# antoniorizzoeng/climate-sim-mpi-cpp

Hardware: AMD Instinct MI355X
Metric: Mcell-updates/sec (16384^2 fp64 advection-diffusion sweep) (higher is better)
Workload: dtype f64

## Files before the change

### climate-sim-mpi-cpp_amd/csrc/api.cpp

```cpp
#include "stepper.hpp"

namespace csim {

static thread_local std::string g_err;
int fail(int code, const std::string& msg) {
    g_err = msg;
    return code;
}
static bool pow2(double x) {
    if (!(x > 0.0) || !std::isnormal(x)) return false;
    int e = 0;
    return std::frexp(x, &e) == 0.5 && std::isnormal(1.0 / x);
}

Phys make_phys(double dx, double dy, double D, double dt, double vx, double vy, bool contract) {
    Phys p;
    p.kdiff = dt * D;
    p.mdt = -dt;
    p.vx = vx;
    p.vy = vy;
    p.dx = dx;
    p.dy = dy;
    p.dx2 = dx * dx;
    p.dy2 = dy * dy;
    p.rdx = 1.0 / dx;
    p.rdy = 1.0 / dy;
    p.rdx2 = 1.0 / p.dx2;
    p.rdy2 = 1.0 / p.dy2;
    if (dx == 1.0 && dy == 1.0)
        p.div_mode = 0;
    else if (pow2(dx) && pow2(dy) && pow2(p.dx2) && pow2(p.dy2))
        p.div_mode = 1;
    else
        p.div_mode = 2;
    {
        const long double kx = static_cast<long double>(dt) * D / (static_cast<long double>(dx) * dx);
        const long double ky = static_cast<long double>(dt) * D / (static_cast<long double>(dy) * dy);
        const long double cx = static_cast<long double>(dt) * vx / dx, cy = static_cast<long double>(dt) * vy / dy;
        const long double acx = cx < 0 ? -cx : cx, acy = cy < 0 ? -cy : cy;
        p.a0 = static_cast<double>(1.0L - 2.0L * kx - 2.0L * ky - acx - acy);
        p.aW = static_cast<double>(kx + (vx >= 0.0 ? acx : 0.0L));
        p.aE = static_cast<double>(kx + (vx >= 0.0 ? 0.0L : acx));
        p.aS = static_cast<double>(ky + (vy >= 0.0 ? acy : 0.0L));
        p.aN = static_cast<double>(ky + (vy >= 0.0 ? 0.0L : acy));
    }
    {
        const double g = (1.0 + 4.0 * std::fabs(p.kdiff) * (1.0 / p.dx2 + 1.0 / p.dy2) +
                          2.0 * std::fabs(p.mdt) * (std::fabs(vx) / std::fabs(dx) + std::fabs(vy) / std::fabs(dy))) * (1.0 + 1e-9);
        const double thr = std::ldexp(1.0, 1022) / std::pow(g, MAX_FUSE);
        p.fast_thr = (std::isfinite(g) && thr >= std::ldexp(1.0, 900)) ? thr : 0.0;
    }
    p.slow_thr = p.p2_hi = p.p2_q = p.p2_k = 0.0;
    if (!contract && p.div_mode <= 1 && p.fast_thr > 0.0 && pow2(std::fabs(vx)) && pow2(std::fabs(vy)) && std::isfinite(p.kdiff) &&
        std::isfinite(p.mdt)) {
        const double A = p.div_mode == 1 ? vx * p.rdx : vx, B = p.div_mode == 1 ? vy * p.rdy : vy;
        if (pow2(std::fabs(A)) && pow2(std::fabs(B))) {
            const bool by_y = vy > 0.0 || vx < 0.0;
            const double q = by_y ? A / B : B / A, K = p.mdt * (by_y ? B : A);
            const int eA = std::ilogb(A), eB = std::ilogb(B), eq = std::ilogb(q);
            int e2 = 0, ew = std::min({0, eA, eB, eq, -eq}), eh = std::max({0, eA, eB, eq, -eq});
            if (p.div_mode == 1) {
                e2 = std::min({0, std::ilogb(p.rdx2), std::ilogb(p.rdy2)});
                ew = std::min({ew, e2, std::ilogb(p.rdx), std::ilogb(p.rdy)});
                eh = std::max({eh, std::ilogb(p.rdx), std::ilogb(p.rdy)});
            }
            int er = 0;
            if (p.kdiff != 0.0) er = std::min(er, std::ilogb(p.kdiff) - 52 + e2);
            if (p.mdt != 0.0) er = std::min(er, std::ilogb(p.mdt) - 52 + std::min(eA, eB));
            const int eL = -1074 + 52 - MAX_FUSE * er - ew;
            if (eL <= -300 && eh <= 100 && pow2(std::fabs(q)) && (K == 0.0 || std::isnormal(K))) {
                p.slow_thr = std::ldexp(1.0, eL);
                p.p2_hi = std::ldexp(p.fast_thr, -(eh + 2));
                p.p2_q = q;
                p.p2_k = K;
            }
        }
    }
    if (contract) p.div_mode = 3;
    return p;
}

int fold_partials(const double* scratch_dev, int rows, int kind, double* out, hipStream_t st, const Members& mb) {
    const size_t G = static_cast<size_t>(reduce_blocks(rows, mb.cap)), hi = G * mb.count;
    std::vector<double> h(kind == 0 ? 2 * hi : hi);
    CSIM_HIP(hipMemcpyAsync(h.data(), scratch_dev, sizeof(double) * h.size(), hipMemcpyDeviceToHost, st));
    CSIM_HIP(hipStreamSynchronize(st));
    for (int m = 0; m < mb.count; ++m) {
        const double* p = h.data() + m * G;
        double r0 = p[0], r1 = kind == 0 ? p[hi] : 0.0;
        for (size_t k = 1; k < G; ++k) {
            if (kind == 0) {
                r0 = std::fmin(r0, p[k]);
                r1 = std::fmax(r1, p[hi + k]);
            } else if (kind == 1) {
                r0 += p[k];
            } else {
                r0 = max_nan(r0, p[k]);
            }
        }
        if (kind == 0) {
            out[2 * m] = r0;
            out[2 * m + 1] = r1;
        } else {
            out[m] = r0;
        }
    }
    return CSIM_OK;
}

int fold_checksum(const double* scratch_dev, int rows, unsigned long long* out, hipStream_t st, const Members& mb) {
    const size_t G = static_cast<size_t>(reduce_blocks(rows, mb.cap));
    std::vector<unsigned long long> h(G * mb.count);
    CSIM_HIP(hipMemcpyAsync(h.data(), scratch_dev, sizeof(unsigned long long) * h.size(), hipMemcpyDeviceToHost, st));
    CSIM_HIP(hipStreamSynchronize(st));
    for (int m = 0; m < mb.count; ++m) {
        unsigned long long acc = 0;
        for (size_t k = 0; k < G; ++k) acc += h[m * G + k];
        out[m] = acc;
    }
    return CSIM_OK;
}

int upload_2d(double* d, int nx, int ny, int pitch, const double* host) {
    CSIM_HIP(hipMemcpy2D(d + (LPAD - 1), sizeof(double) * pitch, host, sizeof(double) * (nx + 2),
                         sizeof(double) * (nx + 2), ny + 2, hipMemcpyHostToDevice));
    return CSIM_OK;
}
int download_2d(const double* d, int nx, int ny, int pitch, double* host) {
    CSIM_HIP(hipMemcpy2D(host, sizeof(double) * (nx + 2), d + (LPAD - 1), sizeof(double) * pitch,
                         sizeof(double) * (nx + 2), ny + 2, hipMemcpyDeviceToHost));
    return CSIM_OK;
}
int download_interior_2d(const double* d, int nx, int ny, int pitch, double* host) {
    CSIM_HIP(hipMemcpy2D(host, sizeof(double) * nx, d + pitch + LPAD, sizeof(double) * pitch,
                         sizeof(double) * nx, ny, hipMemcpyDeviceToHost));
    return CSIM_OK;
}

void neighbours8(const csim_decomp& dec, int nbr8[8]) {
    for (int k = 0; k < 4; ++k) nbr8[k] = dec.nbr[k];
    const int cx = dec.coords[0], cy = dec.coords[1], py = dec.dims[1];
    auto diag = [&](int sx, int sy, int dx_, int dy_) {
        if (dec.nbr[sx] < 0 || dec.nbr[sy] < 0) return -1;
        return dec.size == 1 ? 0 : (cx + dx_) * py + (cy + dy_);
    };
    nbr8[4] = diag(CSIM_LEFT, CSIM_BOTTOM, -1, -1);
    nbr8[5] = diag(CSIM_RIGHT, CSIM_BOTTOM, +1, -1);
    nbr8[6] = diag(CSIM_LEFT, CSIM_TOP, -1, +1);
    nbr8[7] = diag(CSIM_RIGHT, CSIM_TOP, +1, +1);
}

size_t face_doubles(int d, int H, int nx, int ny) {
    if (H == 1) return d < 2 ? static_cast<size_t>(ny) : static_cast<size_t>(nx);
    return d < 2 ? static_cast<size_t>(H) * (ny + 2) : d < 4 ? static_cast<size_t>(H) * (nx + 2)
                                                       : static_cast<size_t>(H) * H;
}

bool valid_bc(const int bc[4]) {
    for (int s = 0; s < 4; ++s)
        if (bc[s] < CSIM_BC_DIRICHLET || bc[s] > CSIM_BC_PERIODIC) return false;
    return true;
}

}

using namespace csim;

extern "C" {

const char* csim_last_error(void) { return g_err.c_str(); }

int csim_abi_version(void) { return CSIM_ABI_VERSION; }

int csim_device_count(int* count) {
    CSIM_REQUIRE(count, "count is null");
    CSIM_HIP(hipGetDeviceCount(count));
    return CSIM_OK;
}

int csim_set_device(int device) {
    CSIM_HIP(hipSetDevice(device));
    return CSIM_OK;
}

int csim_device_name(char* buf, size_t n) {
    CSIM_REQUIRE(buf && n > 0, "bad buffer");
    int dev = 0;
    CSIM_HIP(hipGetDevice(&dev));
    hipDeviceProp_t prop;
    CSIM_HIP(hipGetDeviceProperties(&prop, dev));
    std::snprintf(buf, n, "%s", prop.gcnArchName);
    return CSIM_OK;
}

int csim_pow2_velocity_screen(double dx, double dy, double D, double dt, double vx, double vy, double out[4]) {
    CSIM_REQUIRE(out, "null argument");
    const Phys p = make_phys(dx, dy, D, dt, vx, vy);
    out[0] = p.slow_thr, out[1] = p.p2_hi, out[2] = p.p2_q, out[3] = p.p2_k;
    return CSIM_OK;
}

double csim_safe_dt(double dx, double dy, double vx, double vy, double D) {
    const double inf = std::numeric_limits<double>::infinity();
    const double ax = std::fabs(vx), ay = std::fabs(vy);
    const double rate = (ax > 0 ? ax / dx : 0.0) + (ay > 0 ? ay / dy : 0.0);
    const double dt_adv = rate > 0 ? 1.0 / rate : inf;
    const double w = 1.0 / (dx * dx) + 1.0 / (dy * dy);
    const double dt_diff = D > 0 ? 1.0 / (2.0 * D * w) : inf;
    return std::min(dt_adv, dt_diff);
}

int csim_decomp_init(int size, int rank, int nx_global, int ny_global, csim_decomp* out) {
    CSIM_REQUIRE(out, "out is null");
    CSIM_REQUIRE(size >= 1 && rank >= 0 && rank < size, "bad size/rank");
    CSIM_REQUIRE(nx_global > 0 && ny_global > 0, "nx/ny must be > 0");
    int small = 1;
    for (int f = 1; static_cast<long>(f) * f <= size; ++f)
        if (size % f == 0) small = f;
    csim_decomp d{};
    d.size = size;
    d.rank = rank;
    d.dims[0] = size / small;
    d.dims[1] = small;
    d.coords[0] = rank / d.dims[1];
    d.coords[1] = rank % d.dims[1];
    const int cx = d.coords[0], cy = d.coords[1];
    d.nbr[CSIM_LEFT] = cx > 0 ? (cx - 1) * d.dims[1] + cy : CSIM_NO_NEIGHBOR;
    d.nbr[CSIM_RIGHT] = cx + 1 < d.dims[0] ? (cx + 1) * d.dims[1] + cy : CSIM_NO_NEIGHBOR;
    d.nbr[CSIM_BOTTOM] = cy > 0 ? cx * d.dims[1] + (cy - 1) : CSIM_NO_NEIGHBOR;
    d.nbr[CSIM_TOP] = cy + 1 < d.dims[1] ? cx * d.dims[1] + (cy + 1) : CSIM_NO_NEIGHBOR;
    d.nx_global = nx_global;
    d.ny_global = ny_global;
    const int bx = nx_global / d.dims[0], by = ny_global / d.dims[1];
    d.nx_local = bx + (cx == d.dims[0] - 1 ? nx_global % d.dims[0] : 0);
    d.ny_local = by + (cy == d.dims[1] - 1 ? ny_global % d.dims[1] : 0);
    d.x_offset = cx * bx;
    d.y_offset = cy * by;
    CSIM_REQUIRE(d.nx_local > 0 && d.ny_local > 0, "more ranks than cells along an axis");
    *out = d;
    return CSIM_OK;
}

int csim_exchange_plan(const csim_decomp* dec, int depth, csim_msg sends[8], int* nsend, csim_msg recvs[8],
                       int* nrecv) {
    CSIM_REQUIRE(dec && sends && nsend && recvs && nrecv, "null argument");
    CSIM_REQUIRE(depth >= 1 && depth <= MAX_FUSE, "depth must be 1..7");
    static const int recv_order1[4] = {CSIM_RIGHT, CSIM_LEFT, CSIM_TOP, CSIM_BOTTOM};
    static const int recv_order8[8] = {1, 0, 3, 2, 7, 6, 5, 4};
    int nbr8[8];
    neighbours8(*dec, nbr8);
    const int ndir = depth == 1 ? 4 : 8;
    const int* order = depth == 1 ? recv_order1 : recv_order8;
    int ns = 0, nr = 0;
    for (int d = 0; d < ndir; ++d)
        if (nbr8[d] >= 0)
            sends[ns++] = csim_msg{nbr8[d], d, static_cast<long>(face_doubles(d, depth, dec->nx_local, dec->ny_local))};
    for (int q = 0; q < ndir; ++q) {
        const int d = order[q];
        if (nbr8[d] >= 0)
            recvs[nr++] = csim_msg{nbr8[d], d, static_cast<long>(face_doubles(d, depth, dec->nx_local, dec->ny_local))};
    }
    *nsend = ns;
    *nrecv = nr;
    return CSIM_OK;
}

struct FieldMem : csim_field {
    DeviceBuf mem, partials;
    void release() { mem.release(), partials.release(); }
};
static FieldMem* owner(csim_field* f) { return static_cast<FieldMem*>(f); }

static int field_alloc(FieldMem* f) {
    CSIM_TRY(f->mem.reserve(f->bytes()));
    CSIM_HIP(hipMemset(f->mem.p, 0, f->bytes()));
    CSIM_TRY(f->partials.reserve(sizeof(double) * 2 * REDUCE_BLOCKS));
    f->alloc = f->mem.as();
    f->d = f->alloc + static_cast<size_t>(GHOST_EXTRA) * f->pitch;
    f->scratch = f->partials.as();
    return CSIM_OK;
}

int csim_field_create(int nx, int ny, int halo, double dx, double dy, csim_field** out) {
    CSIM_REQUIRE(out, "out is null");
    *out = nullptr;
    CSIM_REQUIRE(nx > 0 && ny > 0, "nx/ny must be > 0");
    CSIM_REQUIRE(halo == 1, "only halo == 1 is supported (reference src/main.cpp:65)");
    CSIM_REQUIRE(dx > 0 && dy > 0, "dx/dy must be > 0");
    FieldMem* f = new FieldMem;
    f->nx = nx;
    f->ny = ny;
    f->halo = halo;
    f->dx = dx;
    f->dy = dy;
    f->pitch = pitch_for(nx);
    if (field_alloc(f) != CSIM_OK) {
        const std::string why = g_err;
        csim_field_destroy(f);
        return fail(CSIM_ERR_HIP, "csim_field_create: " + why);
    }
    *out = f;
    return CSIM_OK;
}

int csim_field_destroy(csim_field* f) {
    if (!f) return CSIM_OK;
    owner(f)->release();
    delete owner(f);
    return CSIM_OK;
}

int csim_field_upload(csim_field* f, const double* host) {
    CSIM_REQUIRE(f && host, "null argument");
    return upload_2d(f->d, f->nx, f->ny, f->pitch, host);
}

int csim_field_download(const csim_field* f, double* host) {
    CSIM_REQUIRE(f && host, "null argument");
    return download_2d(f->d, f->nx, f->ny, f->pitch, host);
}

int csim_field_download_interior(const csim_field* f, double* host) {
    CSIM_REQUIRE(f && host, "null argument");
    return download_interior_2d(f->d, f->nx, f->ny, f->pitch, host);
}

int csim_field_fill(csim_field* f, double value) {
    CSIM_REQUIRE(f, "null field");
    CSIM_HIP(launch_fill(f->d, f->nx, f->ny, f->pitch, value, nullptr));
    CSIM_HIP(hipStreamSynchronize(nullptr));
    return CSIM_OK;
}

static bool same_shape(const csim_field* a, const csim_field* b) {
    return a && b && a->nx == b->nx && a->ny == b->ny;
}

int csim_field_copy(csim_field* dst, const csim_field* src) {
    CSIM_REQUIRE(same_shape(dst, src), "fields differ in shape");
    CSIM_HIP(hipMemcpy(dst->alloc, src->alloc, src->bytes(), hipMemcpyDeviceToDevice));
    return CSIM_OK;
}

int csim_field_swap(csim_field* a, csim_field* b) {
    CSIM_REQUIRE(same_shape(a, b), "fields differ in shape");
    std::swap(owner(a)->mem, owner(b)->mem);
    std::swap(a->alloc, b->alloc);
    std::swap(a->d, b->d);
    return CSIM_OK;
}

int csim_field_minmax(const csim_field* f, double out[2]) {
    CSIM_REQUIRE(f && out, "null argument");
    CSIM_HIP(launch_minmax(f->d, f->nx, f->ny, f->pitch, f->scratch, nullptr));
    return fold_partials(f->scratch, f->ny + 2, 0, out, nullptr);
}

int csim_field_sum(const csim_field* f, double* out) {
    CSIM_REQUIRE(f && out, "null argument");
    CSIM_HIP(launch_sum(f->d, f->nx, f->ny, f->pitch, f->scratch, nullptr));
    return fold_partials(f->scratch, f->ny, 1, out, nullptr);
}

int csim_field_linf_diff(const csim_field* a, const csim_field* b, double* out) {
    CSIM_REQUIRE(same_shape(a, b) && out, "fields differ in shape");
    CSIM_HIP(launch_linf(a->d, b->d, a->nx, a->ny, a->pitch, a->scratch, nullptr));
    return fold_partials(a->scratch, a->ny, 2, out, nullptr);
}

int csim_apply_boundary(csim_field* f, const int bc[4], const int is_physical[4], double value) {
    CSIM_REQUIRE(f && bc && is_physical, "null argument");
    CSIM_REQUIRE(valid_bc(bc), "unknown boundary type");
    GhostArgs g{};
    for (int s = 0; s < 4; ++s) {
        g.bc[s] = bc[s];
        g.phys[s] = is_physical[s] != 0;
        g.recv[s] = nullptr;
    }
    g.value = value;
    CSIM_HIP(launch_ghost_fill(f->d, nullptr, f->nx, f->ny, f->pitch, g, nullptr));
    CSIM_HIP(hipStreamSynchronize(nullptr));
    return CSIM_OK;
}

int csim_diffusion_step(const csim_field* u, csim_field* out, double D, double dt) {
    CSIM_REQUIRE(same_shape(u, out), "fields differ in shape");
    CSIM_REQUIRE(u->d != out->d, "u and out must be distinct fields");
    const Phys p = make_phys(u->dx, u->dy, D, dt, 0.0, 0.0);
    CSIM_HIP(launch_diffusion_only(u->d, out->d, u->nx, u->ny, u->pitch, p, nullptr));
    CSIM_HIP(launch_ring_copy(u->d, out->d, u->nx, u->ny, u->pitch, nullptr));
    CSIM_HIP(hipStreamSynchronize(nullptr));
    return CSIM_OK;
}

int csim_advection_step(const csim_field* u, csim_field* out, double vx, double vy, double dt) {
    CSIM_REQUIRE(same_shape(u, out), "fields differ in shape");
    CSIM_REQUIRE(u->d != out->d, "u and out must be distinct fields");
    const Phys p = make_phys(u->dx, u->dy, 0.0, dt, vx, vy);
    CSIM_HIP(launch_advection_only(u->d, out->d, u->nx, u->ny, u->pitch, p, nullptr));
    CSIM_HIP(hipStreamSynchronize(nullptr));
    return CSIM_OK;
}

int csim_fused_step(const csim_field* u, csim_field* out, double D, double dt, double vx, double vy) {
    CSIM_REQUIRE(same_shape(u, out), "fields differ in shape");
    CSIM_REQUIRE(u->d != out->d, "u and out must be distinct fields");
    const Phys p = make_phys(u->dx, u->dy, D, dt, vx, vy);
    SweepCfg cfg;
    CSIM_HIP(launch_ring_copy(u->d, out->d, u->nx, u->ny, u->pitch, nullptr));
    CSIM_HIP(launch_sweep(u->d, out->d, u->nx, u->ny, u->pitch, p, cfg, nullptr));
    CSIM_HIP(hipStreamSynchronize(nullptr));
    return CSIM_OK;
}

}
```

### climate-sim-mpi-cpp_amd/csrc/sweepO.hpp

```cpp
#pragma once
#include "sweep_core.hpp"

#pragma clang fp contract(off)

namespace csim {

__device__ __forceinline__ void face_store_cell(const FrameSync& fs, int i, int j, double v, int nx, int ny) {
    const int H = fs.face_depth;
    const unsigned long long bits = static_cast<unsigned long long>(__double_as_longlong(v));
    auto put = [&](double* face, int idx) {
        __hip_atomic_store(reinterpret_cast<unsigned long long*>(face + idx), bits, __ATOMIC_RELAXED, __HIP_MEMORY_SCOPE_AGENT);
    };
    const bool in_i = i >= 1 && i <= nx, in_j = j >= 1 && j <= ny;
    const bool l = in_i && i <= H, r = in_i && i >= nx - H + 1, b = in_j && j <= H, t = in_j && j >= ny - H + 1;
    const int cl = i - 1, cr = i - (nx - H + 1), rb = j - 1, rt = j - (ny - H + 1);
    if (l && fs.face[0]) put(fs.face[0], cl * (ny + 2) + j);
    if (r && fs.face[1]) put(fs.face[1], cr * (ny + 2) + j);
    if (b && fs.face[2]) put(fs.face[2], rb * (nx + 2) + i);
    if (t && fs.face[3]) put(fs.face[3], rt * (nx + 2) + i);
    if (l && b && fs.face[4]) put(fs.face[4], rb * H + cl);
    if (r && b && fs.face[5]) put(fs.face[5], rb * H + cr);
    if (l && t && fs.face[6]) put(fs.face[6], rt * H + cl);
    if (r && t && fs.face[7]) put(fs.face[7], rt * H + cr);
}

#ifdef CSIM_TRACE
__device__ unsigned long long* g_wave_trace = nullptr;
struct WaveTrace {
    int slot, lane;
    unsigned long long t0;
    __device__ WaveTrace(int s, int l) : slot(s), lane(l), t0(wall_clock64()) {}
    __device__ ~WaveTrace() {
        if (lane == 0 && g_wave_trace) {
            g_wave_trace[3 * slot] = t0;
            g_wave_trace[3 * slot + 1] = wall_clock64();
            g_wave_trace[3 * slot + 2] = (static_cast<unsigned long long>(__builtin_amdgcn_s_getreg(63508)) << 32) |
                                         static_cast<unsigned>(__builtin_amdgcn_s_getreg(63492));
        }
    }
};
#endif

template <int DIV, int T, int SX, int SY>
__global__ __launch_bounds__(256) void k_sweepO_dpp(const double* __restrict__ in, double* __restrict__ out, SweepArgs a) {
    constexpr int TP = OverlapGeom<T>::TP;
    constexpr int STRIDE = OverlapGeom<T>::STRIDE;
    const int nx = a.nx, ny = a.ny, pitch = a.pitch, nstrips = a.nstrips;
    const LateArgs late = LateArgs::get();
    const int lane = threadIdx.x & 63;
    const int wave = __builtin_amdgcn_readfirstlane(threadIdx.x >> 6);
#ifdef CSIM_TRACE
    WaveTrace trace_scope(blockIdx.x * 4 + wave, lane);
#endif
    int tile;
    bool frame_tile = false;
    {
        const int b = blockIdx.x;
        if (b < a.tl.frame_blocks) {
            tile = 4 * b + wave;
            if (tile >= a.tl.frame_tiles) return;
            frame_tile = true;
        } else {
            const int lb = b - a.tl.frame_blocks, nb_mid = gridDim.x - a.tl.frame_blocks - a.tl.tail_blocks;
            tile = a.tl.frame_tiles + (lb < nb_mid ? xcd_remap(lb, nb_mid, a.swz) : lb) * 4 + wave;
        }
    }
    if (tile >= a.tl.ntiles) return;
    int t0 = 0, strip0 = a.tl.r[0].strip0, nstrip = a.tl.r[0].nstrip, j0 = a.tl.r[0].j0, j1 = a.tl.r[0].j1, ry = a.tl.r[0].ry;
#pragma unroll
    for (int q = 1; q < 8; ++q)
        if (q < a.tl.nregions && tile >= a.tl.r[q - 1].t_end) {
            t0 = a.tl.r[q - 1].t_end;
            strip0 = a.tl.r[q].strip0, nstrip = a.tl.r[q].nstrip, j0 = a.tl.r[q].j0, j1 = a.tl.r[q].j1, ry = a.tl.r[q].ry;
        }
    const int local = tile - t0;
    const int strip = strip0 + local % nstrip;
    const int chunk = local / nstrip;
    const bool first = strip == 0, last = strip == nstrips - 1;
    const int jb = j0 + chunk * ry;
    const int je = min(jb + ry - 1, j1);
    const int g0 = strip * STRIDE - TP;
    const int kl = first ? a.bc.kind[CSIM_LEFT] : 3;
    const int kr = g0 + WAVE_COLS > nx ? a.bc.kind[CSIM_RIGHT] : 3;
    const int kb = a.bc.kind[CSIM_BOTTOM], kt = a.bc.kind[CSIM_TOP];
    const bool fin_frame = a.fin.line[CSIM_BOTTOM] != nullptr && (first || last || jb == 1 || je == ny);
    const bool edge = kl != 3 || kr != 3 || (kb != 3 && jb - (T - 1) < 1) || (kt != 3 && je + (T - 1) > ny) || fin_frame;
    if (frame_tile && a.fs.prio) __builtin_amdgcn_s_setprio(3);
    const bool signalling = frame_tile && a.fs.flag != nullptr;
    const bool wt = signalling && a.fs.fence == 0;
    if (edge) {
        __builtin_amdgcn_s_setprio(3);
        const bool rows = (kb != 3 && jb - (T - 1) < 1) || (kt != 3 && je + (T - 1) > ny);
        int col_case = 0;
        if (kl != 3 && kr != 3)
            col_case = 7;
        else if (kl != 3)
            col_case = kl == CSIM_BC_NEUMANN ? 2 : 1;
        else if (kr != 3)
            col_case = (kr == CSIM_BC_NEUMANN ? 5 : 3) + (nx & 1);
        if (!SPECIALISE_EDGES<DIV, T>::value || rows || col_case == 7) col_case = -1;
#define CSIM_MARCH(MODE_) \
    sweepO_march<DIV, T, MODE_, SX, SY>(in, out, nx, ny, pitch, jb, je, g0, lane, kl, kr, a.p, kb, kt, late, fin_frame, first, last, wt)
        switch (col_case) {
            case 0: if (SPECIALISE_EDGES<DIV, T>::value) CSIM_MARCH(0); break;
            case 1: if (SPECIALISE_EDGES<DIV, T>::value) CSIM_MARCH(1); break;
            case 2: if (SPECIALISE_EDGES<DIV, T>::value) CSIM_MARCH(2); break;
            case 3: if (SPECIALISE_EDGES<DIV, T>::value) CSIM_MARCH(3); break;
            case 4: if (SPECIALISE_EDGES<DIV, T>::value) CSIM_MARCH(4); break;
            case 5: if (SPECIALISE_EDGES<DIV, T>::value) CSIM_MARCH(5); break;
            case 6: if (SPECIALISE_EDGES<DIV, T>::value) CSIM_MARCH(6); break;
            default: CSIM_MARCH(M_GENERIC); break;
        }
    } else {
        bool redo = true;
        if (DIV != 3 && a.p.fast_thr > 0.0) {
            if constexpr (P2_BODY<DIV, T, SX, SY>::value) {
                if (a.p.slow_thr > 0.0) {
                    keep_branch();
                    redo = CSIM_MARCH(M_FAST_P2);
                } else {
                    redo = CSIM_MARCH(M_FAST);
                }
            } else {
                redo = CSIM_MARCH(M_FAST);
            }
        }
        if (redo) {
            keep_branch();
            CSIM_MARCH(M_PLAIN);
        }
    }
#undef CSIM_MARCH
    if (signalling) {
        const LateArgs::Ptr ka = late.here();
        FrameSync fs;
        fs.counter = ka->fs.counter, fs.flag = ka->fs.flag, fs.pass = ka->fs.pass, fs.nframe = ka->fs.nframe;
        fs.fence = ka->fs.fence, fs.face_depth = ka->fs.face_depth;
#pragma unroll
        for (int d = 0; d < 8; ++d) fs.face[d] = ka->fs.face[d];
        if (fs.fence == 0)
            asm volatile("s_waitcnt vmcnt(0)" ::: "memory");
        if (fs.fence == 0 && fs.face_depth > 0) {
            const int H = fs.face_depth;
            const int gx = g0 + 2 * lane;
            const bool out_lane = 2 * lane >= TP && 2 * lane < TP + STRIDE && gx < nx;
            const bool rows_near = jb <= H || je >= ny - H + 1;
            const bool cols_near = g0 + TP < H || g0 + TP + STRIDE > nx - H;
            if (rows_near || cols_near) {
                const int jf0 = jb == 1 ? 0 : jb, jf1 = je == ny ? ny + 1 : je;
                auto ldf = [&](const double* q) {
                    return __longlong_as_double(static_cast<long long>(__hip_atomic_load(
                        reinterpret_cast<const unsigned long long*>(q), __ATOMIC_RELAXED, __HIP_MEMORY_SCOPE_AGENT)));
                };
                for (int rho = jf0; rho <= jf1; ++rho) {
                    if (!out_lane) continue;
                    const double* src = out + static_cast<ptrdiff_t>(rho) * pitch + LPAD + gx;
                    face_store_cell(fs, gx + 1, rho, ldf(src), nx, ny);
                    if (gx + 1 < nx) face_store_cell(fs, gx + 2, rho, ldf(src + 1), nx, ny);
                    if (gx == 0) face_store_cell(fs, 0, rho, ldf(src - 1), nx, ny);
                    if (gx + 1 == nx) face_store_cell(fs, nx + 1, rho, ldf(src + 1), nx, ny);
                    if (gx + 2 == nx) face_store_cell(fs, nx + 1, rho, ldf(src + 2), nx, ny);
                }
                asm volatile("s_waitcnt vmcnt(0)" ::: "memory");
            }
        }
        if (fs.fence == 1) __threadfence();
        if (lane == 0) {
            const unsigned done = atomicAdd(fs.counter, 1u);
            if (done == fs.nframe - 1) {
                atomicExch(fs.counter, 0u);
                __hip_atomic_store(fs.flag, fs.pass, __ATOMIC_RELEASE, __HIP_MEMORY_SCOPE_SYSTEM);
            }
        }
    }
}


template <int DIV, int T>
hipError_t sweepO_div(const double* in, double* out, int pitch, const Phys& p, const SweepCfg& cfg, const Bc2& bc,
                      const FinLines& fin, const SweepPlan& plan, hipStream_t st, FrameSync fs) {
    if (plan.empty) return hipSuccess;
    if (plan.signals)
        fs.nframe = plan.nframe;
    else
        fs = FrameSync{};
    const dim3 grid(plan.nblocks), block(256);
    SweepArgs ka;
    ka.nx = plan.nx, ka.ny = plan.ny, ka.pitch = pitch, ka.nstrips = plan.nstrips, ka.swz = cfg.xcd_swizzle;
    ka.tl = plan.tl, ka.p = p, ka.bc = bc, ka.fin = fin, ka.fs = fs;
#define CSIM_LAUNCH_O(SXV, SYV) \
    hipLaunchKernelGGL((k_sweepO_dpp<DIV, T, SXV, SYV>), grid, block, cfg.lds_bytes, st, in, out, ka)
#ifdef CSIM_ISA_PROBE
    CSIM_LAUNCH_O(1, 1);
#else
    if (DIV == 3) {
        CSIM_LAUNCH_O(1, 1);
    } else {
        switch (sign_class(p)) {
            case 8: if constexpr (DIV <= 1) CSIM_LAUNCH_O(2, 2); break;
            case 7: if constexpr (DIV <= 1) CSIM_LAUNCH_O(2, 1); break;
            case 6: if constexpr (DIV <= 1) CSIM_LAUNCH_O(2, 0); break;
            case 5: if constexpr (DIV <= 1) CSIM_LAUNCH_O(1, 2); break;
            case 2: if constexpr (DIV <= 1) CSIM_LAUNCH_O(0, 2); break;
            case 4: CSIM_LAUNCH_O(1, 1); break;
            case 3: CSIM_LAUNCH_O(1, 0); break;
            case 1: CSIM_LAUNCH_O(0, 1); break;
            default: CSIM_LAUNCH_O(0, 0); break;
        }
    }
#endif
#undef CSIM_LAUNCH_O
    return hipGetLastError();
}

template <int T>
hipError_t sweepO_T(const double* in, double* out, int pitch, const Phys& p, const SweepCfg& cfg, const Bc2& bc,
                    const FinLines& fin, const SweepPlan& plan, hipStream_t st, const FrameSync& fs) {
#ifdef CSIM_ISA_PROBE
    if (p.div_mode != 0) return hipErrorInvalidValue;
    return sweepO_div<0, T>(in, out, pitch, p, cfg, bc, fin, plan, st, fs);
#else
    switch (p.div_mode) {
        case 0: return sweepO_div<0, T>(in, out, pitch, p, cfg, bc, fin, plan, st, fs);
        case 1: return sweepO_div<1, T>(in, out, pitch, p, cfg, bc, fin, plan, st, fs);
        case 3: return sweepO_div<3, T>(in, out, pitch, p, cfg, bc, fin, plan, st, fs);
        default: return sweepO_div<2, T>(in, out, pitch, p, cfg, bc, fin, plan, st, fs);
    }
#endif
}

}
```

### climate-sim-mpi-cpp_amd/csrc/sweep_core.hpp

```cpp
#pragma once
#include <algorithm>
#include <type_traits>

#include "internal.hpp"

#pragma clang fp contract(off)

namespace csim {

template <int DIV, bool FAST = false>
__device__ __forceinline__ double diffuse_term(double c, double W, double E, double S, double N,
                                               const Phys& p) {
    double lx, ly;
    if (FAST) {
        lx = __builtin_fma(-2.0, c, E) + W;
        ly = __builtin_fma(-2.0, c, N) + S;
    } else {
        const double tc = 2.0 * c;
        lx = (E - tc) + W;
        ly = (N - tc) + S;
    }
    if (DIV == 1) {
        lx = lx * p.rdx2;
        ly = ly * p.rdy2;
    } else if (DIV == 2) {
        lx = lx / p.dx2;
        ly = ly / p.dy2;
    }
    const double lap = lx + ly;
    return c + p.kdiff * lap;
}

template <int DIV, int SX = -1, int SY = -1>
__device__ __forceinline__ double advect_term(double c, double W, double E, double S, double N,
                                              const Phys& p) {
    double gx, gy;
    if (SX == 1)
        gx = c - W;
    else if (SX == 0)
        gx = E - c;
    else
        gx = (p.vx >= 0.0) ? (c - W) : (E - c);
    if (SY == 1)
        gy = c - S;
    else if (SY == 0)
        gy = N - c;
    else
        gy = (p.vy >= 0.0) ? (c - S) : (N - c);
    if (DIV == 1) {
        gx = gx * p.rdx;
        gy = gy * p.rdy;
    } else if (DIV == 2) {
        gx = gx / p.dx;
        gy = gy / p.dy;
    }
    const double adv = p.vx * gx + p.vy * gy;
    return p.mdt * adv;
}

template <int DIV, int SX = -1, int SY = -1, bool FAST = false, bool P2 = false>
__device__ __forceinline__ double cell(double c, double W, double E, double S, double N,
                                       const Phys& p) {
    if (DIV == 3) {
        double o = p.a0 * c;
        o = __builtin_fma(p.aW, W, o);
        o = __builtin_fma(p.aE, E, o);
        o = __builtin_fma(p.aS, S, o);
        return __builtin_fma(p.aN, N, o);
    }
    const double o = diffuse_term<DIV, FAST>(c, W, E, S, N, p);
    if (P2) {
        static_assert(!P2 || (FAST && DIV <= 1 && (SX == 0 || SX == 1) && (SY == 0 || SY == 1)), "see P2 above");
        const double gx = SX == 1 ? c - W : E - c;
        const double gy = SY == 1 ? c - S : N - c;
        const double F = (SY == 1 || SX == 0) ? __builtin_fma(p.p2_q, gx, gy) : __builtin_fma(p.p2_q, gy, gx);
        return o + p.p2_k * F;
    }
    if (FAST && (SX == 2 || SY == 2)) {
        if (SX == 2 && SY == 2) return o;
        double g;
        if (SY == 2)
            g = SX == 1 ? c - W : E - c;
        else
            g = SY == 1 ? c - S : N - c;
        if (DIV == 1) g = g * (SY == 2 ? p.rdx : p.rdy);
        const double adv = (SY == 2 ? p.vx : p.vy) * g;
        return o + p.mdt * adv;
    }
    return o + advect_term<DIV, (SX == 2 ? 1 : SX), (SY == 2 ? 1 : SY)>(c, W, E, S, N, p);
}

__device__ __forceinline__ double from_prev_lane(double src, double edge) {
    int lo = __builtin_amdgcn_update_dpp(__double2loint(edge), __double2loint(src), 0x138, 0xf, 0xf, false);
    int hi = __builtin_amdgcn_update_dpp(__double2hiint(edge), __double2hiint(src), 0x138, 0xf, 0xf, false);
    return __hiloint2double(hi, lo);
}
__device__ __forceinline__ double from_next_lane(double src, double edge) {
    int lo = __builtin_amdgcn_update_dpp(__double2loint(edge), __double2loint(src), 0x130, 0xf, 0xf, false);
    int hi = __builtin_amdgcn_update_dpp(__double2hiint(edge), __double2hiint(src), 0x130, 0xf, 0xf, false);
    return __hiloint2double(hi, lo);
}

__device__ __forceinline__ int xcd_remap(int b, int nb, int enable) {
    if (!enable || nb < 16) return b;
    const int per = nb >> 3, rem = nb & 7;
    const int xcd = b & 7, q = b >> 3;
    return xcd < rem ? xcd * (per + 1) + q : rem * (per + 1) + (xcd - rem) * per + q;
}

__device__ __forceinline__ void store_pair_wt(double* dst, double ox, double oy, int nvalid) {
    if (nvalid >= 1)
        __hip_atomic_store(reinterpret_cast<unsigned long long*>(dst), static_cast<unsigned long long>(__double_as_longlong(ox)),
                           __ATOMIC_RELAXED, __HIP_MEMORY_SCOPE_AGENT);
    if (nvalid >= 2)
        __hip_atomic_store(reinterpret_cast<unsigned long long*>(dst + 1), static_cast<unsigned long long>(__double_as_longlong(oy)),
                           __ATOMIC_RELAXED, __HIP_MEMORY_SCOPE_AGENT);
}

__device__ __forceinline__ void store_pair(double* dst, double ox, double oy, int nvalid) {
    if (nvalid >= 2) {
        *reinterpret_cast<double2*>(dst) = make_double2(ox, oy);
    } else if (nvalid == 1) {
        dst[0] = ox;
    }
}

struct Bc2 {
    int kind[4];
    double value;
};

__device__ __forceinline__ double shift_from_prev(double src) {
    int lo = __builtin_amdgcn_update_dpp(0, __double2loint(src), 0x138, 0xf, 0xf, true);
    int hi = __builtin_amdgcn_update_dpp(0, __double2hiint(src), 0x138, 0xf, 0xf, true);
    return __hiloint2double(hi, lo);
}
__device__ __forceinline__ double shift_from_next(double src) {
    int lo = __builtin_amdgcn_update_dpp(0, __double2loint(src), 0x130, 0xf, 0xf, true);
    int hi = __builtin_amdgcn_update_dpp(0, __double2hiint(src), 0x130, 0xf, 0xf, true);
    return __hiloint2double(hi, lo);
}

__device__ __forceinline__ void keep_branch() { asm volatile(""); }

struct FinLines {
    double* line[4];
};

struct SweepArgs {
    int nx, ny, pitch, nstrips, swz;
    Tiling tl;
    Phys p;
    Bc2 bc;
    FinLines fin;
    FrameSync fs;
};
constexpr int SWEEP_ARGS_KERNARG_OFFSET = 16;
static_assert(alignof(SweepArgs) <= 8 && 2 * sizeof(void*) == SWEEP_ARGS_KERNARG_OFFSET,
              "LateArgs reads SweepArgs from the kernel-argument segment right behind the two field pointers");

struct LateArgs {
    typedef const SweepArgs __attribute__((address_space(4))) * Ptr;
    Ptr a;
    __device__ __forceinline__ static LateArgs get() {
        typedef const char __attribute__((address_space(4))) * Bytes;
        LateArgs l;
        l.a = (Ptr)((Bytes)__builtin_amdgcn_kernarg_segment_ptr() + SWEEP_ARGS_KERNARG_OFFSET);
        return l;
    }
    __device__ __forceinline__ Ptr here() const {
        Ptr q = a;
        asm volatile("" : "+s"(q));
        return q;
    }
    __device__ __forceinline__ double* fin_line(int side) const { return here()->fin.line[side]; }
};

template <int T>
struct OverlapGeom {
    static constexpr int TP = strip_overlap(T);
    static constexpr int STRIDE = strip_stride(T);
};

__device__ __forceinline__ void pin(double& v) { asm volatile("" : "+v"(v)); }
__device__ __forceinline__ void pin2(double2& v) { asm volatile("" : "+v"(v.x), "+v"(v.y)); }

constexpr int M_FAST_P2 = -4, M_FAST = -3, M_PLAIN = -2, M_GENERIC = -1;

template <int DIV, int T, int MODE, int SX, int SY>
__device__ __forceinline__ bool sweepO_march(const double* __restrict__ in, double* __restrict__ out,
                                             int nx, int ny, int pitch, int jb, int je, int g0, int lane,
                                             int kl, int kr, const Phys& p, int kb, int kt,
                                             LateArgs late, bool fin_any, bool fin_l, bool fin_r, bool wt) {
    constexpr int TP = OverlapGeom<T>::TP;
    constexpr int STRIDE = OverlapGeom<T>::STRIDE;
    constexpr bool EDGE = MODE >= M_GENERIC, P2 = MODE == M_FAST_P2, FAST = MODE == M_FAST || P2, GENERIC = MODE == M_GENERIC;
    constexpr int CASE = MODE;
    const int gx = g0 + 2 * lane, gy = gx + 1;
    const ptrdiff_t xoff = LPAD + gx;
    const bool out_lane = 2 * lane >= TP && 2 * lane < TP + STRIDE && gx < nx;
    const int nvalid = nx - gx;
    const bool ghost_ly = kl != 3 && gy == -1;
    const bool ghost_rx = kr != 3 && gx == nx, ghost_ry = kr != 3 && gy == nx;
    const bool right_in_x = (nx & 1) == 0;
    const bool ghost_cols = kl != 3 || kr != 3;

    auto load = [&](int j) {
        return *reinterpret_cast<const double2*>(in + static_cast<ptrdiff_t>(j) * pitch + xoff);
    };

    const int r_first = jb - (T - 1);
    const int niter = (je - jb + 1) + 2 * (T - 1);
    const int last_row = r_first + niter;
    double2 L0[6];
    double2 L[T][3];
#pragma unroll
    for (int q = 0; q < 6; ++q) L0[q] = load(min(r_first - 1 + q, last_row));
    bool big = false;
    auto screen = [&](const double2& v) {
        big |= !(__builtin_fabs(v.x) < (P2 ? p.p2_hi : p.fast_thr));
        big |= !(__builtin_fabs(v.y) < (P2 ? p.p2_hi : p.fast_thr));
        if (P2) {
            big |= __builtin_fabs(v.x) < p.slow_thr && v.x != 0.0;
            big |= __builtin_fabs(v.y) < p.slow_thr && v.y != 0.0;
        }
        if (SX == 2 || SY == 2 || (P2 && SX == 0 && SY == 0)) {
            big |= __builtin_amdgcn_class(v.x, 0x20);
            big |= __builtin_amdgcn_class(v.y, 0x20);
        }
    };
    if (FAST) {
        screen(L0[0]);
        screen(L0[1]);
    }
#pragma unroll
    for (int l = 0; l < T; ++l)
#pragma unroll
        for (int q = 0; q < 3; ++q) L[l][q] = make_double2(0.0, 0.0);

    auto group = [&](auto gtag, int k0) {
        constexpr int G = decltype(gtag)::value;
        const bool rows_here = GENERIC && ((kb != 3 && k0 <= 2 * T - 2 - jb) || (kt != 3 && k0 + 5 >= ny + T - jb));
#pragma unroll
        for (int u = 0; u < 6; ++u) {
            {
                const int r = r_first + k0 + u;
#pragma unroll
                for (int l = 1; l <= T; ++l) {
                    if (G < 2 && 6 * G + u < 2 * (l - 1)) continue;
                    const int rho = r - l + 1;
                    const double2 s = (l == 1) ? L0[u % 6] : L[l - 1][(u + 1) % 3];
                    const double2 c = (l == 1) ? L0[(u + 1) % 6] : L[l - 1][(u + 2) % 3];
                    const double2 n = (l == 1) ? L0[(u + 2) % 6] : L[l - 1][u % 3];
                    double2 o;
                    {
                        const double Wx = shift_from_prev(c.y);
                        const double Ey = shift_from_next(c.x);
                        o.x = cell<DIV, SX, SY, FAST, P2>(c.x, Wx, c.y, s.x, n.x, p);
                        o.y = cell<DIV, SX, SY, FAST, P2>(c.y, c.x, Ey, s.y, n.y, p);
                        if (FAST && l == 1) screen(n);
                    }
                    if (EDGE && !GENERIC && l < T) {
                        if (CASE == 1) o.y = ghost_ly ? c.y : o.y;
                        if (CASE == 2) {
                            const double nb = shift_from_next(o.x);
                            o.y = ghost_ly ? nb : o.y;
                        }
                        if (CASE == 3) o.x = ghost_rx ? c.x : o.x;
                        if (CASE == 4) o.y = ghost_ry ? c.y : o.y;
                        if (CASE == 5) {
                            const double pb = shift_from_prev(o.y);
                            o.x = ghost_rx ? pb : o.x;
                        }
                        if (CASE == 6) o.y = ghost_ry ? o.x : o.y;
                    }
                    if (GENERIC && l < T) {
                        bool ghost_row = false;
                        if (rows_here) {
                            const bool gb = rho == 0 && kb != 3, gt = rho == ny + 1 && kt != 3;
                            ghost_row = gb || gt;
                            if (ghost_row) {
                                const int kk = gb ? kb : kt;
                                if (kk != CSIM_BC_NEUMANN) {
                                    double2 t = c;
                                    pin2(t);
                                    o = t;
                                } else if (gt) {
                                    double2 t = L[l][(u + 2) % 3];
                                    pin2(t);
                                    o = t;
                                }
                            }
                        }
                        if (!ghost_row && ghost_cols) {
                            if (kl == CSIM_BC_NEUMANN) {
                                double t = o.x;
                                pin(t);
                                const double nb = shift_from_next(t);
                                o.y = ghost_ly ? nb : o.y;
                            } else if (kl != 3) {
                                double t = c.y;
                                pin(t);
                                o.y = ghost_ly ? t : o.y;
                            }
                            if (kr == CSIM_BC_NEUMANN) {
                                if (right_in_x) {
                                    double t = o.y;
                                    pin(t);
                                    const double pb = shift_from_prev(t);
                                    o.x = ghost_rx ? pb : o.x;
                                } else {
                                    double t = o.x;
                                    pin(t);
                                    o.y = ghost_ry ? t : o.y;
                                }
                            } else if (kr != 3) {
                                if (right_in_x) {
                                    double t = c.x;
                                    pin(t);
                                    o.x = ghost_rx ? t : o.x;
                                } else {
                                    double t = c.y;
                                    pin(t);
                                    o.y = ghost_ry ? t : o.y;
                                }
                            }
                        }
                    }
                    if (EDGE && T >= 2 && l == T - 1 && fin_any) {
                        keep_branch();
                        if (rho >= jb && rho <= je) {
                            if (fin_l && (kl != 3 ? gx == 0 : gy == -1)) late.fin_line(CSIM_LEFT)[rho - 1] = kl != 3 ? o.x : o.y;
                            if (fin_r) {
                                const int col = kr != 3 ? nx - 1 : nx;
                                if (gx == col) late.fin_line(CSIM_RIGHT)[rho - 1] = o.x;
                                if (gy == col) late.fin_line(CSIM_RIGHT)[rho - 1] = o.y;
                            }
                        }
                        if (jb == 1 && rho == (kb != 3 ? 1 : 0) && out_lane) store_pair(late.fin_line(CSIM_BOTTOM) + gx, o.x, o.y, nvalid);
                        if (je == ny && rho == (kt != 3 ? ny : ny + 1) && out_lane) store_pair(late.fin_line(CSIM_TOP) + gx, o.x, o.y, nvalid);
                    }
                    if (l < T) {
                        if (GENERIC && rows_here && rho == 1 && kb == CSIM_BC_NEUMANN) {
                            double2 t = o;
                            pin2(t);
                            L[l][(u + 2) % 3] = t;
                        }
                        L[l][u % 3] = o;
                    } else if (rho >= jb && rho <= je && out_lane) {
                        if (wt) {
                            keep_branch();
                            store_pair_wt(out + static_cast<ptrdiff_t>(rho) * pitch + xoff, o.x, o.y, nvalid);
                        } else {
                            store_pair(out + static_cast<ptrdiff_t>(rho) * pitch + xoff, o.x, o.y, nvalid);
                        }
                    }
                }
                L0[u % 6] = load(min(r + 5, last_row));
            }
        }
    };
    using G2 = std::integral_constant<int, 2>;
    if (EDGE) {
        for (int k0 = 0; k0 < niter; k0 += 6) group(G2{}, k0);
    } else {
        group(std::integral_constant<int, 0>{}, 0);
        if (niter > 6) group(std::integral_constant<int, 1>{}, 6);
        for (int k0 = 12; k0 < niter; k0 += 6) group(G2{}, k0);
    }
    return FAST && __builtin_amdgcn_ballot_w64(big) != 0;
}

template <int DIV, int T>
struct SPECIALISE_EDGES {
    static constexpr bool value = specialise_edges(DIV, T);
};

template <int DIV, int T, int SX, int SY>
struct P2_BODY {
    static constexpr bool value = SPECIALISE_EDGES<DIV, T>::value && (SX == 0 || SX == 1) && (SY == 0 || SY == 1);
};

struct GhostDev {
    int bc[4];
    int phys[4];
    double value;
    const double* recv[4];
    const double* adj[4];
    int ext_depth;
};

__device__ __forceinline__ size_t at(int i, int j, int pitch) {
    return static_cast<size_t>(j) * pitch + (LPAD - 1) + i;
}

__device__ __forceinline__ void ghost_fill_cell(double* __restrict__ a, double* __restrict__ b, int nx, int ny,
                                                int pitch, const GhostDev& g, int t) {
    auto put = [&](size_t o, double v) {
        a[o] = v;
        if (b) b[o] = v;
    };
    if (t < ny) {
        const int j = t + 1;
        for (int s = CSIM_LEFT; s <= CSIM_RIGHT; ++s) {
            const int ig = s == CSIM_LEFT ? 0 : nx + 1;
            const int ia = s == CSIM_LEFT ? 1 : nx;
            if (g.phys[s]) {
                if (g.bc[s] == CSIM_BC_DIRICHLET)
                    put(at(ig, j, pitch), g.value);
                else if (g.bc[s] == CSIM_BC_NEUMANN)
                    put(at(ig, j, pitch), g.adj[s] ? g.adj[s][t] : a[at(ia, j, pitch)]);
            } else if (g.recv[s]) {
                put(at(ig, j, pitch), g.recv[s][t]);
            }
        }
    }
    if (t < nx) {
        const int i = t + 1;
        for (int s = CSIM_BOTTOM; s <= CSIM_TOP; ++s) {
            const int jg = s == CSIM_BOTTOM ? 0 : ny + 1;
            const int ja = s == CSIM_BOTTOM ? 1 : ny;
            if (g.phys[s]) {
                if (g.bc[s] == CSIM_BC_DIRICHLET)
                    put(at(i, jg, pitch), g.value);
                else if (g.bc[s] == CSIM_BC_NEUMANN)
                    put(at(i, jg, pitch), g.adj[s] ? g.adj[s][t] : a[at(i, ja, pitch)]);
            } else if (g.recv[s]) {
                put(at(i, jg, pitch), g.recv[s][t]);
            }
        }
    }
    const int tc = nx > ny ? nx : ny;
    if (t == tc) {
        for (int cs = CSIM_LEFT; cs <= CSIM_RIGHT; ++cs) {
            const int ig = cs == CSIM_LEFT ? 0 : nx + 1;
            const int ia = cs == CSIM_LEFT ? 1 : nx;
            for (int rs = CSIM_BOTTOM; rs <= CSIM_TOP; ++rs) {
                const int jg = rs == CSIM_BOTTOM ? 0 : ny + 1;
                const int ja = rs == CSIM_BOTTOM ? 1 : ny;
                const bool row_d = g.phys[rs] && g.bc[rs] == CSIM_BC_DIRICHLET;
                const bool row_n = g.phys[rs] && g.bc[rs] == CSIM_BC_NEUMANN;
                const bool col_d = g.phys[cs] && g.bc[cs] == CSIM_BC_DIRICHLET;
                const bool col_n = g.phys[cs] && g.bc[cs] == CSIM_BC_NEUMANN;
                if (row_d) {
                    put(at(ig, jg, pitch), g.value);
                } else if (row_n) {
                    double v;
                    if (col_d)
                        v = g.value;
                    else if (col_n)
                        v = g.adj[cs] ? g.adj[cs][ja - 1] : a[at(ia, ja, pitch)];
                    else if (!g.phys[cs] && g.recv[cs])
                        v = g.recv[cs][ja - 1];
                    else
                        v = a[at(ig, ja, pitch)];
                    put(at(ig, jg, pitch), v);
                } else if (col_d) {
                    put(at(ig, jg, pitch), g.value);
                } else if (col_n) {
                    double v;
                    if (!g.phys[rs] && g.recv[rs])
                        v = g.recv[rs][ia - 1];
                    else
                        v = a[at(ia, jg, pitch)];
                    put(at(ig, jg, pitch), v);
                }
            }
        }
    }
}

}
```

Before: 1.670 million.

## Screen P2 fast path with integer bit-range accumulators and full-wave vector stores

Result: no change. 1.662 million (-0.5%).

```diff
diff --git a/climate-sim-mpi-cpp_amd/csrc/api.cpp b/climate-sim-mpi-cpp_amd/csrc/api.cpp
--- a/climate-sim-mpi-cpp_amd/csrc/api.cpp
+++ b/climate-sim-mpi-cpp_amd/csrc/api.cpp
@@ -70,7 +70,7 @@
             const int eL = -1074 + 52 - MAX_FUSE * er - ew;
             if (eL <= -300 && eh <= 100 && pow2(std::fabs(q)) && (K == 0.0 || std::isnormal(K))) {
                 p.slow_thr = std::ldexp(1.0, eL);
-                p.p2_hi = std::ldexp(p.fast_thr, -(eh + 2));
+                p.p2_hi = std::ldexp(1.0, std::ilogb(p.fast_thr) - (eh + 2));
                 p.p2_q = q;
                 p.p2_k = K;
             }
diff --git a/climate-sim-mpi-cpp_amd/csrc/p2_screen.hpp b/climate-sim-mpi-cpp_amd/csrc/p2_screen.hpp
--- /dev/null
+++ b/climate-sim-mpi-cpp_amd/csrc/p2_screen.hpp
@@ -0,0 +1,64 @@
+#pragma once
+#include <cstdint>
+#include <cstring>
+
+#if defined(__HIPCC__) || defined(__CUDACC__)
+#define CSIM_HD __host__ __device__ __forceinline__
+#else
+#define CSIM_HD inline
+#endif
+
+namespace csim {
+
+struct P2Acc {
+    uint32_t tmin;
+    int32_t smax;
+    uint32_t umax;
+    int32_t smin;
+};
+
+CSIM_HD P2Acc p2_acc_init() { return P2Acc{0xffffffffu, 0, 0u, 0}; }
+
+CSIM_HD uint64_t p2_bits(double v) {
+#if defined(__HIP_DEVICE_COMPILE__)
+    return static_cast<uint64_t>(__double_as_longlong(v));
+#else
+    uint64_t b;
+    std::memcpy(&b, &v, sizeof b);
+    return b;
+#endif
+}
+
+CSIM_HD uint32_t p2_min3(uint32_t a, uint32_t b, uint32_t c) { return (a < b ? a : b) < c ? (a < b ? a : b) : c; }
+CSIM_HD uint32_t p2_max3(uint32_t a, uint32_t b, uint32_t c) { return (a > b ? a : b) > c ? (a > b ? a : b) : c; }
+CSIM_HD int32_t p2_min3(int32_t a, int32_t b, int32_t c) { return (a < b ? a : b) < c ? (a < b ? a : b) : c; }
+CSIM_HD int32_t p2_max3(int32_t a, int32_t b, int32_t c) { return (a > b ? a : b) > c ? (a > b ? a : b) : c; }
+
+template <bool NEG0>
+CSIM_HD void p2_acc_pair(P2Acc& a, double x, double y) {
+    const uint64_t bx = p2_bits(x), by = p2_bits(y);
+    const uint32_t hx = static_cast<uint32_t>(bx >> 32), hy = static_cast<uint32_t>(by >> 32);
+    const uint32_t tx = static_cast<uint32_t>(((bx << 1) - 1) >> 32), ty = static_cast<uint32_t>(((by << 1) - 1) >> 32);
+    a.tmin = p2_min3(a.tmin, tx, ty);
+    a.smax = p2_max3(a.smax, static_cast<int32_t>(hx), static_cast<int32_t>(hy));
+    a.umax = p2_max3(a.umax, hx, hy);
+    if (NEG0) a.smin = p2_min3(a.smin, static_cast<int32_t>(hx), static_cast<int32_t>(hy));
+}
+
+template <bool NEG0>
+CSIM_HD bool p2_rejects(const P2Acc& a, double slow_thr, double p2_hi) {
+    const uint32_t lo2 = static_cast<uint32_t>((p2_bits(slow_thr) << 1) >> 32);
+    const uint32_t hi = static_cast<uint32_t>(p2_bits(p2_hi) >> 32);
+    bool bad = a.tmin < lo2 || a.smax >= static_cast<int32_t>(hi) || a.umax >= (0x80000000u | hi);
+    if (NEG0) bad = bad || a.smin == INT32_MIN;
+    return bad;
+}
+
+template <bool NEG0>
+CSIM_HD bool p2_accepts(double v, double slow_thr, double p2_hi) {
+    P2Acc a = p2_acc_init();
+    p2_acc_pair<NEG0>(a, v, 0.0);
+    return !p2_rejects<NEG0>(a, slow_thr, p2_hi);
+}
+
+}
diff --git a/climate-sim-mpi-cpp_amd/csrc/sweepO.hpp b/climate-sim-mpi-cpp_amd/csrc/sweepO.hpp
--- a/climate-sim-mpi-cpp_amd/csrc/sweepO.hpp
+++ b/climate-sim-mpi-cpp_amd/csrc/sweepO.hpp
@@ -113,18 +113,30 @@
         }
     } else {
         bool redo = true;
+        const bool full = g0 + WAVE_COLS <= nx && !wt;
+#define CSIM_MARCH_FULL(MODE_) \
+    sweepO_march<DIV, T, MODE_, SX, SY, true>(in, out, nx, ny, pitch, jb, je, g0, lane, kl, kr, a.p, kb, kt, late, fin_frame, first, last, false)
         if (DIV != 3 && a.p.fast_thr > 0.0) {
-            if constexpr (P2_BODY<DIV, T, SX, SY>::value) {
-                if (a.p.slow_thr > 0.0) {
+            bool p2 = false;
+            if constexpr (P2_BODY<DIV, T, SX, SY>::value) p2 = a.p.slow_thr > 0.0;
+            if (p2) {
+                if constexpr (P2_BODY<DIV, T, SX, SY>::value) {
                     keep_branch();
-                    redo = CSIM_MARCH(M_FAST_P2);
-                } else {
-                    redo = CSIM_MARCH(M_FAST);
+                    if (full) {
+                        keep_branch();
+                        redo = CSIM_MARCH_FULL(M_FAST_P2);
+                    } else {
+                        redo = CSIM_MARCH(M_FAST_P2);
+                    }
                 }
+            } else if (full) {
+                keep_branch();
+                redo = CSIM_MARCH_FULL(M_FAST);
             } else {
                 redo = CSIM_MARCH(M_FAST);
             }
         }
+#undef CSIM_MARCH_FULL
         if (redo) {
             keep_branch();
             CSIM_MARCH(M_PLAIN);
diff --git a/climate-sim-mpi-cpp_amd/csrc/sweep_core.hpp b/climate-sim-mpi-cpp_amd/csrc/sweep_core.hpp
--- a/climate-sim-mpi-cpp_amd/csrc/sweep_core.hpp
+++ b/climate-sim-mpi-cpp_amd/csrc/sweep_core.hpp
@@ -3,6 +3,7 @@
 #include <type_traits>
 
 #include "internal.hpp"
+#include "p2_screen.hpp"
 
 #pragma clang fp contract(off)
 
@@ -187,7 +188,7 @@
 
 constexpr int M_FAST_P2 = -4, M_FAST = -3, M_PLAIN = -2, M_GENERIC = -1;
 
-template <int DIV, int T, int MODE, int SX, int SY>
+template <int DIV, int T, int MODE, int SX, int SY, bool FULL = false>
 __device__ __forceinline__ bool sweepO_march(const double* __restrict__ in, double* __restrict__ out,
                                              int nx, int ny, int pitch, int jb, int je, int g0, int lane,
                                              int kl, int kr, const Phys& p, int kb, int kt,
@@ -217,14 +218,16 @@
 #pragma unroll
     for (int q = 0; q < 6; ++q) L0[q] = load(min(r_first - 1 + q, last_row));
     bool big = false;
+    constexpr bool P2_NEG0 = P2 && SX == 0 && SY == 0;
+    P2Acc p2acc = p2_acc_init();
     auto screen = [&](const double2& v) {
-        big |= !(__builtin_fabs(v.x) < (P2 ? p.p2_hi : p.fast_thr));
-        big |= !(__builtin_fabs(v.y) < (P2 ? p.p2_hi : p.fast_thr));
         if (P2) {
-            big |= __builtin_fabs(v.x) < p.slow_thr && v.x != 0.0;
-            big |= __builtin_fabs(v.y) < p.slow_thr && v.y != 0.0;
-        }
-        if (SX == 2 || SY == 2 || (P2 && SX == 0 && SY == 0)) {
+            p2_acc_pair<P2_NEG0>(p2acc, v.x, v.y);
+            return;
+        }
+        big |= !(__builtin_fabs(v.x) < p.fast_thr);
+        big |= !(__builtin_fabs(v.y) < p.fast_thr);
+        if (SX == 2 || SY == 2) {
             big |= __builtin_amdgcn_class(v.x, 0x20);
             big |= __builtin_amdgcn_class(v.y, 0x20);
         }
@@ -348,7 +351,9 @@
                         }
                         L[l][u % 3] = o;
                     } else if (rho >= jb && rho <= je && out_lane) {
-                        if (wt) {
+                        if (FULL) {
+                            *reinterpret_cast<double2*>(out + static_cast<ptrdiff_t>(rho) * pitch + xoff) = o;
+                        } else if (wt) {
                             keep_branch();
                             store_pair_wt(out + static_cast<ptrdiff_t>(rho) * pitch + xoff, o.x, o.y, nvalid);
                         } else {
@@ -367,6 +372,10 @@
         group(std::integral_constant<int, 0>{}, 0);
         if (niter > 6) group(std::integral_constant<int, 1>{}, 6);
         for (int k0 = 12; k0 < niter; k0 += 6) group(G2{}, k0);
+    }
+    if (P2) {
+        const LateArgs::Ptr ka = late.here();
+        big = p2_rejects<P2_NEG0>(p2acc, ka->p.slow_thr, ka->p.p2_hi);
     }
     return FAST && __builtin_amdgcn_ballot_w64(big) != 0;
 }
```
